# Stalfoes/dqn_mgsc_zoo

Hardware: AMD Instinct MI355X
Metric: learner grad-steps/sec at batch=32, 84×84×4 uint8, 1/2/4/8 MI355X (higher is better)
Workload: dtype f32

## Files before the change

### dqn_mgsc_zoo_amd/_native.py

```python

import ctypes
import glob
import hashlib
import os
import threading

_HERE = os.path.dirname(os.path.abspath(__file__))
LIB_PATH = os.environ.get('DQZ_LIB') or os.path.join(_HERE, 'libdqz.so')
HEADER_PATH = os.path.join(os.path.dirname(_HERE), 'include', 'dqz.h')

DQZ_OK = 0
ALGO_DQN = 0
ALGO_DOUBLE = 1
ALGO_PER = 2
NUM_LEAVES = 10
NUM_PHASES = 10
PHASE_NAMES = (
    'conv1_fwd', 'conv2_fwd', 'conv3_fwd', 'fc1_fwd', 'head', 'fc1_dx',
    'conv3_dx+conv2_dx+fc1_dw+conv3_dw+conv2_dw+conv1_dw', 'unused7',
    'unused8', 'update')
FRAME_H = 84
FRAME_W = 84
STACK = 4
FRAME_BYTES = FRAME_H * FRAME_W
# ... 159 lines not shown
        _int,
        [_vp, ctypes.POINTER(DqzParams), ctypes.POINTER(DqzStore), _vp, _vp,
         ctypes.c_uint64, _vp, _vp, _vp, _vp]),
    'dqz_learner_step_per_draw': (
        _int,
        [_vp, ctypes.POINTER(DqzParams), ctypes.POINTER(DqzStore),
         ctypes.POINTER(DqzPerDraw), _vp]),
    'dqz_learner_grad': (
        _int,
        [_vp, ctypes.POINTER(DqzParams), ctypes.POINTER(DqzStore), _vp, _vp,
         _vp, _vp],
    ),
    'dqz_learner_outputs': (_int, [_vp, _vp, _vp, _vp, _vp]),
    'dqz_learner_sync_status': (_int, [_vp, _vp]),
    'dqz_learner_debug_stall': (_int, [_vp, _int, ctypes.c_uint]),
    'dqz_learner_debug_activations': (_int, [_vp, _int] + [_vp] * 10),
    'dqz_per_write_back': (_int, [_vp, _vp, _i64, _vp, ctypes.c_double, _vp, _vp]),
    'dqz_learner_profile': (
        _int,
        [_vp, ctypes.POINTER(DqzParams), ctypes.POINTER(DqzStore), _vp, _vp,
         _int, ctypes.POINTER(ctypes.c_float), _vp],
    ),
    'dqz_forward': (_int, [_vp, _vp, _vp, _int, _vp, _vp]),
    'dqz_forward_slots': (
        _int, [_vp, _vp, ctypes.POINTER(DqzStore), _vp, _int, _int, _vp, _vp]),
    'dqz_act': (
        _int, [_vp, _vp, _vp, _int, ctypes.c_double, ctypes.c_uint64,
               ctypes.c_uint64, _vp, _vp]),
    'dqz_store_put': (
        _int, [ctypes.POINTER(DqzStore), ctypes.POINTER(DqzTransitionPut), _vp,
# ... 134 lines not shown
```

### dqn_mgsc_zoo_amd/csrc/bwd.hpp

```cpp
#pragma once
#include "common.hpp"
#include "conv1.hpp"
#include "fwd.hpp"
#include "head.hpp"
#include "sampling.hpp"

namespace dqz {

struct Fc1BwdArgs {
  const float* dz1;
  const float* y3;
  float *th, *mu, *nu;
  int64_t w_off;
  Rms rms;
  int B;
  float* dy3;
  const float *w3, *w2;
  float *w3p, *w2p;
};

__device__ __forceinline__ int w3p_src(int i) {
  const int j = i & 3, kq = (i >> 2) & 3, n = (i >> 4) & 15, w = (i >> 8) & 3, r = i >> 10;
  const int tp = r % 9, nq = r / 9;
  return ((8 - tp) * C3CI + 16 * nq + n) * C3CO + 16 * w + 4 * j + kq;
}
__device__ __forceinline__ int w2p_src(int i) {
  const int j = i & 3, kq = (i >> 2) & 3, n = (i >> 4) & 15, w = (i >> 8) & 3, tp = (i >> 10) & 3;
  const int hh = (i >> 12) & 1, pw = (i >> 13) & 1, ph = (i >> 14) & 1;
  const int kh = ph + 2 * (1 - (tp >> 1)), kw = pw + 2 * (1 - (tp & 1));
  return ((kh * C2K + kw) * C2CI + 16 * hh + n) * C2CO + 16 * w + 4 * j + kq;
}
constexpr int W3P_N = 4 * 9 * 1024, W2P_N = 8 * 4 * 1024;

// ... 48 lines not shown
        xacc[mt] = mfma4(av.w, wv[j].w, xacc[mt]);
      }
    }
#pragma unroll
    for (int mt = 0; mt < 2; ++mt)
#pragma unroll
      for (int r = 0; r < 4; ++r) s_red[w][mt][red_at(4 * kq + r, n)] = xacc[mt][r];
    __syncthreads();
#pragma unroll
    for (int h = 0; h < 2; ++h) {
      const int sample = c + 16 * h + (t >> 4);
      const int k = red_at(t >> 4, t & 15);
      const float v2 = (s_red[0][h][k] + s_red[1][h][k]) + (s_red[2][h][k] + s_red[3][h][k]);
      if (sample < a.B) a.dy3[(int64_t)sample * FLAT + k0 + (t & 15)] = ym[h] > 0.f ? v2 : 0.f;
    }
  }
  DQZ_STAMP(5, 3);
}

constexpr int C3X_S = 66, C3X_RS = 754, C3X_WIN = 11 * C3X_RS;
constexpr int C3W_S = 80, C3W_RS = 720, C3W_WIN = 9 * C3W_RS;

struct Conv3BwdArgs {
  const float* dy3;
  const float* y2;
  const float* w3;
  const float* w3p;
  float* dy2;
  float* part;
  int B;
// ... 500 lines not shown
  }
  DQZ_STAMP(11, 3);
}


constexpr int FC1X_BLOCKS = FLAT / 16;
inline int fc1_dx_blocks(int B) { return FC1X_BLOCKS * ((B + 31) / 32); }
__device__ __forceinline__ void fc1_dx_block(const Fc1BwdArgs& a, float* smem, int blk) {
  const int g = blk * 256 + threadIdx.x;
  float v3 = 0.f, v2 = 0.f;
  if (a.w3p) {
    if (g < W3P_N) v3 = a.w3[w3p_src(g)];
    if (g < W2P_N) v2 = a.w2[w2p_src(g)];
  }
  const int kb = blk % FC1X_BLOCKS, c = 32 * (blk / FC1X_BLOCKS);
  fc1_dx_body(a, smem, kb, c, min(c + 32, a.B));
  if (a.w3p) {
    if (g < W3P_N) a.w3p[g] = v3;
    if (g < W2P_N) a.w2p[g] = v2;
  }
  DQZ_STAMP(5, 3);
}

constexpr int FC1X1_ROWS = 32;
constexpr int FC1X1_BLOCKS = FLAT / FC1X1_ROWS;

template <int AMAX, int SMAX, int ZMAX>
__global__ __launch_bounds__(512) void head_dx1_kernel(HeadArgs h, Fc1BwdArgs a) {
  __shared__ __attribute__((aligned(16))) float s_dz[HID];
  DQZ_STAMP(5, 0);
  const int half = threadIdx.x >> 8, t = threadIdx.x & 255;
// ... 22 lines not shown
    d = __fmaf_rn(wv[j].z, z.z, d);
    d = __fmaf_rn(wv[j].w, z.w, d);
  }
  d += dpp_f<0xB1>(d);
  d += dpp_f<0x4E>(d);
  d += dpp_f<0x141>(d);
  d += dpp_f<0x140>(d);
  if ((t & 15) == 0) a.dy3[r] = ym > 0.f ? d : 0.f;
  if (a.w3p) {
    if (g < W3P_N) a.w3p[g] = v3;
    if (g < W2P_N) a.w2p[g] = v2;
  }
  DQZ_STAMP(5, 3);
}

#ifdef DQZ_STEP_TU
inline hipError_t launch_head_dx1(const HeadArgs& h, const Fc1BwdArgs& f, hipStream_t st) {
  if (h.S > 7 || h.Z < 1 || h.Z > 3 || h.B != 1) return hipErrorInvalidValue;
  const dim3 grid(FC1X1_BLOCKS), block(512);
  if (h.A <= 8) {
    if (h.Z <= 2)
      hipLaunchKernelGGL((head_dx1_kernel<8, 7, 2>), grid, block, 0, st, h, f);
    else
      hipLaunchKernelGGL((head_dx1_kernel<8, 7, 3>), grid, block, 0, st, h, f);
  } else {
    if (h.Z <= 2)
      hipLaunchKernelGGL((head_dx1_kernel<MAXA, 7, 2>), grid, block, 0, st, h, f);
    else
      hipLaunchKernelGGL((head_dx1_kernel<MAXA, 7, 3>), grid, block, 0, st, h, f);
  }
  return hipGetLastError();
}
#endif

DQZ_STEP_KERNEL __launch_bounds__(256) void fc1_dx_kernel(Fc1BwdArgs a) {
  __shared__ __attribute__((aligned(16))) float smem[FC1X_SMEM];
  fc1_dx_block(a, smem, blockIdx.x);
}

template <bool WB>
__global__ __launch_bounds__(256) __attribute__((amdgpu_waves_per_eu(4, 8))) void bwd_bc_kernel(
    Conv3BwdArgs c3, Fc1BwdArgs f1, Conv2BwdArgs c2, Conv1DwArgs c1, PerWbArgs wb) {
  constexpr int kW = C3X_WIN > FC1W_SMEM ? C3X_WIN : FC1W_SMEM;
  constexpr int kW2 = C2X_WIN > C3W_WIN ? C2X_WIN : C3W_WIN;
  constexpr int kW3 = C2V_WIN > C1H_SMEM ? C2V_WIN : C1H_SMEM;
  constexpr int kWA = kW > kW2 ? kW : kW2;
  constexpr int kSmem = kWA > kW3 ? kWA : kW3;
  static_assert(kSmem * 4 >= PWB_LDS_BYTES, "the write-back's LDS comes out of the backward's buffer");
  __shared__ __attribute__((aligned(16))) float smem[kSmem];
  const int B8 = (c3.B + 7) / 8 * 8;
// ... 60 lines not shown
```

### dqn_mgsc_zoo_amd/csrc/common.hpp

```cpp
#pragma once
#include <hip/hip_runtime.h>

#include <cstdarg>
#include <cstdint>
#include <cstdio>
#include <string>

#include "dqz.h"

namespace dqz {

typedef float f32x4 __attribute__((ext_vector_type(4)));

#define DQZ_STR(x) #x
#define DQZ_XSTR(x) DQZ_STR(x)
typedef float f32x16 __attribute__((ext_vector_type(16)));

#ifdef DQZ_STEP_TU
#define DQZ_STEP_KERNEL __global__
#define DQZ_OTHER_KERNEL template <int = 0> __global__
#else
#define DQZ_STEP_KERNEL template <int = 0> __global__
#define DQZ_OTHER_KERNEL __global__
#endif
// ... 221 lines not shown
        __builtin_amdgcn_s_sleep(4);
        if (++spins > spin_max) {
          __hip_atomic_fetch_or(err, 1, __ATOMIC_RELAXED, __HIP_MEMORY_SCOPE_AGENT);
          break;
        }
      }
      if (__hip_atomic_fetch_add(ack + b * kStride, 1, __ATOMIC_RELAXED, __HIP_MEMORY_SCOPE_AGENT) == consumers - 1) {
        __hip_atomic_store(cnt + b * kStride, 0, __ATOMIC_RELAXED, __HIP_MEMORY_SCOPE_AGENT);
        __hip_atomic_store(ack + b * kStride, 0, __ATOMIC_RELAXED, __HIP_MEMORY_SCOPE_AGENT);
      }
    }
    __syncthreads();
  }
};

__device__ __forceinline__ float4 load_sc1_f4(const float4* base, int bytes, int e) {
  typedef unsigned u32x4 __attribute__((ext_vector_type(4)));
  const __amdgpu_buffer_rsrc_t r = __builtin_amdgcn_make_buffer_rsrc((void*)base, 0, bytes, 0x00020000);
  return __builtin_bit_cast(float4, __builtin_amdgcn_raw_buffer_load_b128(r, e * 16, 0, 16));
}

__device__ __forceinline__ float load_sc1_f1(const float* base, int bytes, int e) {
  const __amdgpu_buffer_rsrc_t r = __builtin_amdgcn_make_buffer_rsrc((void*)base, 0, bytes, 0x00020000);
  return __builtin_bit_cast(float, __builtin_amdgcn_raw_buffer_load_b32(r, e * 4, 0, 16));
}

__device__ __forceinline__ void store_sc1_f4(float* base, int bytes, int off, f32x4 v) {
  typedef unsigned u32x4 __attribute__((ext_vector_type(4)));
  const __amdgpu_buffer_rsrc_t r = __builtin_amdgcn_make_buffer_rsrc((void*)base, 0, bytes, 0x00020000);
  __builtin_amdgcn_raw_buffer_store_b128(__builtin_bit_cast(u32x4, v), r, off, 0, 16);
// ... 25 lines not shown
```

### dqn_mgsc_zoo_amd/csrc/head.hpp

```cpp
#pragma once
#include "common.hpp"

namespace dqz {

struct HeadArgs {
  const float* fc1p;
  int S;
  float* h1;
  NetZ nz;
  int64_t b1_off, w2_off, b2_off;
  int Z, B, A, algo, shared_bias, fwd_only;
  const int32_t* slots;
  const int32_t* action;
  const float* reward;
  const float* discount;
  const float* weights;
  const double* per_wb;
  int per_normalize;
  float* per_w_out;
  const float* meta_p;
  const float* meta_logits;
  const int32_t* meta_pos;
  int meta_M;
  float *meta_x_out, *meta_p_out;
  const float4* rec;
  uint64_t* advance;
  int unit;
  float bound;
  float* q;
  float* td;
  float* loss_part;
  float* gq;
  int32_t* ga;
  float* dz1;
  dqz_action* act_out;
  double eps;
  uint64_t act_seed, act_ctr;
};

__device__ __forceinline__ dqz_action eps_greedy(const float* q, int A, double eps, double u) {
  float v = q[0];
  for (int a = 1; a < A; ++a) v = fmaxf(v, q[a]);
  int ties = 0;
  for (int a = 0; a < A; ++a) ties += q[a] == v;
  const double greedy = 1.0 / (double)ties, floor = eps / (double)A;
  double total = 0.0;
  for (int a = 0; a < A; ++a) total += (1.0 - eps) * (q[a] == v ? greedy : 0.0) + floor;
  double cum = 0.0;
  int act = A - 1;
// ... 7 lines not shown
  return dqz_action{act, v};
}

__device__ __forceinline__ double wave_max_nonneg(double m) {
  m = fmax(m, dpp_d<0x111>(m));
  m = fmax(m, dpp_d<0x112>(m));
  m = fmax(m, dpp_d<0x114>(m));
  m = fmax(m, dpp_d<0x118>(m));
  m = fmax(m, dpp_d<0x142, 0xa>(m));
  m = fmax(m, dpp_d<0x143, 0xc>(m));
  const long long b = __builtin_bit_cast(long long, m);
  const int lo = __builtin_amdgcn_readlane((int)b, 63), hi = __builtin_amdgcn_readlane((int)(b >> 32), 63);
  return __builtin_bit_cast(double, ((long long)hi << 32) | (unsigned)lo);
}

template <int AMAX, int SMAX, int ZMAX>
__device__ __forceinline__ void head_body(const HeadArgs& h, int b, bool out = true, float* s_dzo = nullptr) {
  DQZ_STAMP(4, 0);
  __shared__ float s_red[8][3 * AMAX];
  __shared__ float s_q[3][AMAX];
  __shared__ float s_rec[5];
  const int n = threadIdx.x, lane = n & 63, wave = n >> 6;
  const int A = h.A, B = h.B, Z = h.Z, S = h.S;
  int a_tm1 = 0;
  float r = 0.f, d = 0.f, w = 1.f, pm = 0.f;
  const bool chain = !h.fwd_only && h.rec == nullptr;
  const int slot = chain ? h.slots[b] : 0;
  float4 rv = make_float4(0.f, 0.f, 0.f, 0.f);
  if (!h.fwd_only && h.rec != nullptr && n == 0) rv = h.rec[b];
  float pv[ZMAX][SMAX], b1v[ZMAX], w2v[ZMAX][AMAX];
#pragma unroll
  for (int z = 0; z < ZMAX; ++z) {
    const int zc = min(z, Z - 1);
    const float* part = h.fc1p + ((int64_t)zc * S * B + b) * HID + n;
#pragma unroll
    for (int s = 0; s < SMAX; ++s) pv[z][s] = part[(int64_t)min(s, S - 1) * B * HID];
    b1v[z] = h.nz.p[zc][h.b1_off + n];
    const float* w2 = h.nz.p[zc] + h.w2_off + n * A;
#pragma unroll
    for (int a = 0; a < AMAX; ++a) w2v[z][a] = w2[min(a, A - 1)];
  }
  constexpr bool kTr = AMAX <= 8;
  constexpr int kPS = HID + 16;
  __shared__ float s_p[kTr ? 3 * AMAX : 1][kTr ? kPS : 1];
  const int K = Z * A, lgT = K <= 16 ? 5 : 4, T = 1 << lgT;
  const int kk = n >> lgT, jj = n & (T - 1);
  const bool qthread = kTr ? (kk < K && jj == 0) : (n < 3 * AMAX && n / AMAX < Z && n % AMAX < A);
  const int zq = kTr ? min(kk / A, 2) : n / AMAX, aq = kTr ? kk % A : n % AMAX;
  float b2v = 0.f;
  {
    const int a2 = h.shared_bias ? 0 : min(aq, A - 1);
    float b2z[ZMAX];
#pragma unroll
    for (int z = 0; z < ZMAX; ++z) b2z[z] = h.nz.p[min(z, Z - 1)][h.b2_off + a2];
    const int zc = min(zq, Z - 1);
#pragma unroll
    for (int z = 0; z < ZMAX; ++z) b2v = zc == z ? b2z[z] : b2v;
  }
  float wper = 1.f;
// ... 67 lines not shown
      if (z == 0) DQZ_STAMP(15, 0);
      if constexpr (kTr) {
#pragma unroll
        for (int a = 0; a < AMAX; ++a)
          if (a < A) s_p[z * A + a][n] = hz[z] * w2v[z][a];
      } else {
#pragma unroll
        for (int a = 0; a < AMAX; ++a) {
          const float sa = wave_sum(hz[z] * w2v[z][a]);
          if (lane == 0) s_red[wave][z * AMAX + a] = sa;
        }
      }
    }
  }
  DQZ_STAMP(15, 1);
  __syncthreads();
  float qv = 0.f;
  if constexpr (kTr) {
    if (kk < K) {
      const float* row = &s_p[kk][jj];
      float a4[4] = {0.f, 0.f, 0.f, 0.f};
      for (int i = 0; i < (HID >> lgT); i += 4) {
#pragma unroll
        for (int u = 0; u < 4; ++u) a4[u] += row[(i + u) << lgT];
      }
      float v = (a4[0] + a4[1]) + (a4[2] + a4[3]);
      v += dpp_f<0xB1>(v);
      v += dpp_f<0x4E>(v);
      v += dpp_f<0x141>(v);
      v += dpp_f<0x140>(v);
// ... 42 lines not shown
          }
        v = q1[0];
#pragma unroll
        for (int a = 1; a < AMAX; ++a) v = a == am ? q1[a] : v;
      }
      const float td = __fmaf_rn(d, v, r) - qa;
      float g;
      if (h.unit) {
        g = -1.f;
      } else if (h.meta_p || h.meta_logits) {
        g = pm * fminf(fmaxf(td, -h.bound), h.bound);
      } else {
        g = w * td / (float)B;
        g = fminf(fmaxf(g, -h.bound), h.bound);
      }
      if (out && n == 0) {
        h.td[b] = td;
        h.loss_part[b] = 0.5f * td * td * w;
        h.gq[b] = -g;
        h.ga[b] = a_tm1;
      }
      float wv = w2v[0][0];
#pragma unroll
      for (int a = 1; a < AMAX; ++a) wv = a == a_tm1 ? w2v[0][a] : wv;
      DQZ_STAMP(4, 2);
      const float dz = hz[0] > 0.f ? -g * wv : 0.f;
      if (s_dzo) s_dzo[n] = dz;
      if (out) h.dz1[(int64_t)b * HID + n] = dz;
    }
  } else if (h.act_out) {
// ... 371 lines not shown
```

### dqn_mgsc_zoo_amd/csrc/learner.hip

```cpp
#include <hip/hip_runtime.h>

#include <algorithm>
#include <array>
#include <functional>
#include <cmath>
#include <vector>
#include <cstdlib>
#include <cstring>

#include "learner_impl.hpp"
#include "meta.hpp"
#include "hvp.hpp"
#include "preprocess.hpp"
#include "census.hpp"

using namespace dqz;

static int g_meta_attr_done = 0;

static int init_meta_attrs() {
  if (g_meta_attr_done) return DQZ_OK;
  DQZ_HIP(hipFuncSetAttribute((const void*)tangent_fwd_kernel, hipFuncAttributeMaxDynamicSharedMemorySize,
                              (int)kConv1FwdSmem));
  g_meta_attr_done = 1;
// ... 1017 lines not shown
  DQZ_HIP(hipGetLastError());
  if (keep) return chunk_sums(logit_buf, logits, true, st);
  return DQZ_OK;
}

int dqz_meta_sync_status(dqz_meta* H, int* status) {
  if (!H || !status) return fail(DQZ_ERR_INVALID, "null argument");
  int s_lm = 0, s_l1 = 0, s_own = 0;
  if (int rc = dqz_learner_sync_status(H->lm, &s_lm)) return rc;
  if (int rc = dqz_learner_sync_status(H->l1, &s_l1)) return rc;
  DQZ_HIP(hipMemcpy(&s_own, H->arrive + 4 * Handoff::kStride, sizeof(int), hipMemcpyDeviceToHost));
  *status = s_lm | s_l1 | s_own;
  if (*status != 0) {
    DQZ_HIP(hipMemset(H->arrive, 0, sizeof(int) * 5 * Handoff::kStride));
    for (dqz_learner* L : {H->lm, H->l1})
      DQZ_HIP(hipMemset(L->sync, 0, sizeof(int) * ((16 * L->cfg.batch + 3) * Handoff::kStride + 64)));
    DQZ_HIP(hipDeviceSynchronize());
  }
  return DQZ_OK;
}

int dqz_meta_debug_stall(dqz_meta* H, int poison, unsigned spin_max) {
  if (!H) return fail(DQZ_ERR_INVALID, "null meta handle");
  const unsigned sm = spin_max ? spin_max : 1u << 24;
  H->spin_max = sm;
  H->lm->spin_max = sm;
  H->l1->spin_max = sm;
  if (poison) {
    const int32_t p = -(1 << 30);
    DQZ_HIP(hipDeviceSynchronize());
    DQZ_HIP(hipMemcpy(H->arrive + Handoff::kStride, &p, sizeof(p), hipMemcpyHostToDevice));
// ... 138 lines not shown
```

### dqn_mgsc_zoo_amd/csrc/learner_impl.hpp

```cpp
#pragma once
#include <hip/hip_runtime.h>

#include <cstring>

#include "common.hpp"
#include "conv1.hpp"
#include "fwd.hpp"
#include "head.hpp"
#include "bwd.hpp"
#include "sampling.hpp"

namespace dqz {

inline void param_layout(int A, int shared_bias, int64_t off[10], int64_t sz[10], int64_t* total) {
  const int64_t sizes[10] = {C1KK * C1CO, C1CO, C2KK * C2CO, C2CO, C3KK * C3CO, C3CO,
                             (int64_t)FLAT * HID, HID, (int64_t)HID * A, shared_bias ? 1 : A};
  int64_t o = 0;
  for (int i = 0; i < 10; ++i) {
    off[i] = o;
    sz[i] = sizes[i];
    o += (sizes[i] + 63) / 64 * 64;
  }
  *total = o;
}

}

struct dqz_learner {
  dqz_learner_config cfg;
  int Z, shared_bias;
  int64_t off[10], sz[10], total;
  int S_fc1, S2, S3;
  float *y1, *y2, *y3, *fc1p, *h1, *q, *dz1, *dy3, *dy2, *dy1, *p1, *p2, *p3, *td, *loss, *loss_part, *gq, *rec;
  float *w3p, *w2p;
  double* per_wb;
  int32_t* ga;
  int32_t* sync;
  unsigned spin_max = 1u << 24;
  void* block;
};


namespace dqz {

inline int check_store(const dqz_store* S) {
  if (!S || !S->frames || !S->fidx || !S->action || !S->reward || !S->discount)
    return fail(DQZ_ERR_INVALID, "store has a null buffer");
  if (S->capacity < 1) return fail(DQZ_ERR_INVALID, "store capacity must be positive");
  return DQZ_OK;
}

inline int device_view(const void* p, const void** out, const char* what) {
  hipPointerAttribute_t attr;
  if (hipPointerGetAttributes(&attr, p) != hipSuccess) {
    (void)hipGetLastError();
    return fail(DQZ_ERR_INVALID, "%s must be device memory or pinned host memory", what);
  }
  if (attr.type == hipMemoryTypeHost) {
// ... 34 lines not shown
```

### dqn_mgsc_zoo_amd/csrc/learner_step.hip

```cpp
#define DQZ_STEP_TU 1
#include <hip/hip_runtime.h>

#include <cstdlib>
#include <cstring>

#include "learner_impl.hpp"

using namespace dqz;

static int g_attr_done = 0;

static int init_kernel_attrs() {
  if (g_attr_done) return DQZ_OK;
  const void* fwd_kernels[] = {(const void*)fwd_conv_kernel<0>, (const void*)fwd_conv_kernel<1>,
                               (const void*)fwd_conv_kernel<2>, (const void*)fwd_conv_kernel<3>,
                               (const void*)fwd_conv_kernel<4>};
  for (const void* k : fwd_kernels)
    DQZ_HIP(hipFuncSetAttribute(k, hipFuncAttributeMaxDynamicSharedMemorySize, (int)kConv1FwdSmem));
  g_attr_done = 1;
  return DQZ_OK;
}

extern "C" {

// ... 15 lines not shown
  L->cfg = *cfg;
  L->Z = cfg->algo == DQZ_ALGO_DQN ? 2 : 3;
  L->shared_bias = cfg->algo == DQZ_ALGO_DQN ? 0 : 1;
  param_layout(cfg->num_actions, L->shared_bias, L->off, L->sz, &L->total);
  const int B = cfg->batch, Z = L->Z, A = cfg->num_actions;
  L->S_fc1 = FC1_S;
  L->S2 = B;
  L->S3 = B;
  const int64_t n_y1 = (int64_t)Z * B * C1M * C1CO, n_y2 = (int64_t)Z * B * C2M * C2CO, n_y3 = (int64_t)Z * B * FLAT;
  const int64_t n_fc1p = (int64_t)Z * L->S_fc1 * B * HID, n_h1 = (int64_t)Z * B * HID, n_q = (int64_t)Z * B * A;
  const int64_t n_dz1 = (int64_t)B * HID, n_dy3 = (int64_t)B * FLAT, n_dy2 = (int64_t)B * C2M * C2CO,
                n_dy1 = (int64_t)B * C1M * C1CO;
  const int64_t n_p1 = (int64_t)B * C1_BLOCKS * (C1KK + 1) * C1CO, n_p2 = (int64_t)L->S2 * (C2KK + 1) * C2CO,
                n_p3 = (int64_t)L->S3 * (C3KK + 1) * C3CO;
  const int64_t sizes[] = {n_y1, n_y2, n_y3, n_fc1p, n_h1, n_q, n_dz1, n_dy3, n_dy2, n_dy1,
                           n_p1, n_p2, n_p3, B,      1,    B,   B,     B,  4 * B, (16 * B + 3) * Handoff::kStride + 64, W3P_N, W2P_N,
                           2 * (int64_t)B};
  float** ptrs[] = {&L->y1,  &L->y2,  &L->y3,  &L->fc1p, &L->h1,   &L->q,         &L->dz1, &L->dy3,
                    &L->dy2, &L->dy1, &L->p1,  &L->p2,   &L->p3,   &L->td,        &L->loss, &L->loss_part,
                    &L->gq,  reinterpret_cast<float**>(&L->ga), &L->rec, reinterpret_cast<float**>(&L->sync), &L->w3p, &L->w2p,
                    reinterpret_cast<float**>(&L->per_wb)};
  static_assert(sizeof(sizes) / sizeof(sizes[0]) == sizeof(ptrs) / sizeof(ptrs[0]), "scratch table");
  int64_t total = 0;
  for (int64_t s : sizes) total += (s + 63) / 64 * 64;
  if (hipMalloc(&L->block, total * sizeof(float)) != hipSuccess) {
    delete L;
    return fail(DQZ_ERR_HIP, "hipMalloc of %lld bytes failed", (long long)(total * 4));
  }
  if (hipMemset(L->block, 0, total * sizeof(float)) != hipSuccess) {
    (void)hipFree(L->block);
    delete L;
    return fail(DQZ_ERR_HIP, "hipMemset of learner scratch failed");
  }
  float* p = (float*)L->block;
  for (size_t i = 0; i < sizeof(sizes) / sizeof(sizes[0]); ++i) {
    *ptrs[i] = p;
// ... 207 lines not shown

  Fc1BwdArgs fb{};
  fb.dz1 = L->dz1;
  fb.y3 = L->y3;
  fb.th = P->online;
  fb.mu = P->mu;
  fb.nu = P->nu;
  fb.w_off = L->off[6];
  fb.rms = rms;
  fb.B = B;
  fb.dy3 = L->dy3;
  fb.w3 = P->online + L->off[4];
  fb.w2 = P->online + L->off[2];
  fb.w3p = L->w3p;
  fb.w2p = L->w2p;
  if (B == 1 && !pe.on()) {
    DQZ_HIP(launch_head_dx1(h, fb, st));
  } else {
    DQZ_PHASE(4, DQZ_HIP(launch_head(h, B, st)));
    DQZ_PHASE(5, hipLaunchKernelGGL(fc1_dx_kernel, dim3(fc1_dx_blocks(B)), dim3(256), 0, st, fb);
              DQZ_HIP(hipGetLastError()));
  }

  Conv3BwdArgs c3b{};
  c3b.dy3 = L->dy3;
  c3b.y2 = L->y2;
  c3b.w3 = P->online + L->off[4];
  c3b.w3p = L->w3p;
  c3b.dy2 = L->dy2;
  c3b.part = L->p3;
  c3b.B = B;
  int* const herr = L->sync + 16 * B * Handoff::kStride;
// ... 106 lines not shown
  for (int i = 0; i < DQZ_NUM_PHASES; ++i) phase_ms[i] = 0.f;
  PhaseEvents pe{nullptr, nullptr, iters, phase_ms};
  DQZ_HIP(hipEventCreate(&pe.e0));
  DQZ_HIP(hipEventCreate(&pe.e1));
  const int rc = step_impl(L, P, S, slots, is_weights, stream, pe);
  (void)hipEventDestroy(pe.e0);
  (void)hipEventDestroy(pe.e1);
  return rc;
}

int dqz_learner_sync_status(dqz_learner* L, int* status) {
  if (!L || !status) return fail(DQZ_ERR_INVALID, "null argument");
  DQZ_HIP(hipDeviceSynchronize());
  DQZ_HIP(hipMemcpy(status, L->sync + 16 * L->cfg.batch * Handoff::kStride, sizeof(int), hipMemcpyDeviceToHost));
  if (*status != 0) {
    DQZ_HIP(hipMemset(L->sync, 0, sizeof(int) * ((16 * L->cfg.batch + 3) * Handoff::kStride + 64)));
    DQZ_HIP(hipDeviceSynchronize());
  }
  return DQZ_OK;
}

int dqz_learner_debug_stall(dqz_learner* L, int sample, unsigned spin_max) {
  if (!L) return fail(DQZ_ERR_INVALID, "null learner");
  if (sample >= L->cfg.batch) return fail(DQZ_ERR_INVALID, "sample out of range");
  L->spin_max = spin_max ? spin_max : 1u << 24;
  if (sample >= 0) {
    const int32_t poison = -(1 << 30);
    DQZ_HIP(hipDeviceSynchronize());
    DQZ_HIP(hipMemcpy(L->sync + (int64_t)sample * Handoff::kStride, &poison, sizeof(poison),
                      hipMemcpyHostToDevice));
  }
  return DQZ_OK;
}

int dqz_learner_outputs(dqz_learner* L, float* q_tm1, float* td, float* loss, void* stream) {
  if (!L) return fail(DQZ_ERR_INVALID, "null learner");
  hipStream_t st = (hipStream_t)stream;
  const int B = L->cfg.batch, A = L->cfg.num_actions;
  if (q_tm1) DQZ_HIP(hipMemcpyAsync(q_tm1, L->q, sizeof(float) * B * A, hipMemcpyDeviceToDevice, st));
  if (td) DQZ_HIP(hipMemcpyAsync(td, L->td, sizeof(float) * B, hipMemcpyDeviceToDevice, st));
  if (loss) DQZ_HIP(hipMemcpyAsync(loss, L->loss, sizeof(float), hipMemcpyDeviceToDevice, st));
  return DQZ_OK;
}

static int forward_q(dqz_learner* L, const float* params, const Conv1Src& src, int which, int n, float* q_out,
                     hipStream_t st) {
// ... 72 lines not shown
```

### dqn_mgsc_zoo_amd/learner.py

```python

import ctypes

import numpy as np
import torch

from dqn_mgsc_zoo_amd import _native
from dqn_mgsc_zoo_amd import networks as networks_lib
from dqn_mgsc_zoo_amd import optim_state

ALGOS = {'dqn': _native.ALGO_DQN, 'double': _native.ALGO_DOUBLE,
         'per': _native.ALGO_PER}


class RMSPropConfig:

  def __init__(self, learning_rate, decay=0.9, eps=1e-8, centered=False):
    if not centered:
      raise NotImplementedError(
          'only centered RMSProp is on the hot path (dqn/run_atari.py:208-213)')
    self.learning_rate = float(learning_rate)
    self.decay = float(decay)
    self.eps = float(eps)
    self.centered = True

# ... 139 lines not shown

  def fetch_outputs(self, stream=None):
    _native.check(_native.lib().dqz_learner_outputs(
        self._h, _native.ptr(self.q_tm1), _native.ptr(self.td),
        _native.ptr(self.loss), _native.stream_handle(stream)))
    return self.q_tm1, self.td, self.loss

  def sync_status(self):
    st = ctypes.c_int(0)
    _native.check(_native.lib().dqz_learner_sync_status(self._h, ctypes.byref(st)))
    return st.value

  def debug_stall(self, sample, spin_max=0):
    _native.check(_native.lib().dqz_learner_debug_stall(self._h, int(sample), int(spin_max)))

  def fetch_activations(self, z=0, backward=False, stream=None):
    b, a = self.batch_size, self.network.num_actions
    shapes = dict(y1=(b, 20, 20, 32), y2=(b, 9, 9, 64), y3=(b, 7, 7, 64),
                  h1=(b, 512), q=(b, a))
    if backward:
      shapes.update(dz1=(b, 512), dy3=(b, 7, 7, 64), dy2=(b, 9, 9, 64),
                    dy1=(b, 20, 20, 32))
    out = {k: torch.empty(s, dtype=torch.float32, device=self.device)
           for k, s in shapes.items()}
    _native.check(_native.lib().dqz_learner_debug_activations(
        self._h, int(z),
        *(_native.ptr(out.get(k)) for k in ('y1', 'y2', 'y3', 'h1', 'q', 'dz1',
                                             'dy3', 'dy2', 'dy1')),
        _native.stream_handle(stream)))
    return out
# ... 188 lines not shown
```

### include/dqz.h

```cpp
#ifndef DQZ_H_
#define DQZ_H_

#include <stdint.h>

#ifdef __cplusplus
extern "C" {
#endif

#define DQZ_OK 0
#define DQZ_ERR_INVALID (-1)
#define DQZ_ERR_HIP (-2)
#define DQZ_ERR_UNSUPPORTED (-3)

#define DQZ_ALGO_DQN 0
#define DQZ_ALGO_DOUBLE 1
#define DQZ_ALGO_PER 2

#define DQZ_FRAME_H 84
#define DQZ_FRAME_W 84
#define DQZ_STACK 4
#define DQZ_FRAME_BYTES (DQZ_FRAME_H * DQZ_FRAME_W)
#define DQZ_NUM_LEAVES 10

const char* dqz_last_error(void);
// ... 58 lines not shown

int dqz_learner_grad(dqz_learner* learner, const dqz_params* params, const dqz_store* store,
                     const int32_t* slots, const float* is_weights, float* grad_out, void* stream);

#define DQZ_NUM_PHASES 10

int dqz_learner_profile(dqz_learner* learner, const dqz_params* params, const dqz_store* store,
                        const int32_t* slots, const float* is_weights, int iters, float* phase_ms,
                        void* stream);

int dqz_learner_outputs(dqz_learner* learner, float* q_tm1, float* td, float* loss, void* stream);

int dqz_learner_sync_status(dqz_learner* learner, int* status);

int dqz_learner_debug_stall(dqz_learner* learner, int sample, unsigned spin_max);

int dqz_learner_debug_activations(dqz_learner* learner, int z, float* y1, float* y2, float* y3, float* h1,
                                  float* q, float* dz1, float* dy3, float* dy2, float* dy1, void* stream);

int dqz_forward(dqz_learner* learner, const float* params, const uint8_t* states, int n,
                float* q_out, void* stream);

int dqz_forward_slots(dqz_learner* learner, const float* params, const dqz_store* store,
                      const int32_t* slots, int n, int which, float* q_out, void* stream);

typedef struct dqz_action {
  int32_t action;
  float value;
} dqz_action;
int dqz_act(dqz_learner* learner, const float* params, const uint8_t* states, int n, double epsilon,
// ... 159 lines not shown
```

Baseline: 16300.

## Merge head and fc1 dx into one kernel with compact dz record handoff

Adds a merged head_dx kernel. The first B workgroups run the head and publish a compact per-sample record (negated grad, action, ReLU mask bits) through an atomic counter handoff. The remaining workgroups rebuild dz1 on the fly from W2 rows and the mask, then compute fc1 dx, so one kernel launch and the dense dz1 round trip are removed. It risks spin-wait deadlock and deliberately pads LDS so only one workgroup fits per CU, which lowers occupancy.

```diff
diff --git a/dqn_mgsc_zoo_amd/_native.py b/dqn_mgsc_zoo_amd/_native.py
--- a/dqn_mgsc_zoo_amd/_native.py
+++ b/dqn_mgsc_zoo_amd/_native.py
@@ -197,6 +197,7 @@
     'dqz_learner_outputs': (_int, [_vp, _vp, _vp, _vp, _vp]),
     'dqz_learner_sync_status': (_int, [_vp, _vp]),
     'dqz_learner_debug_stall': (_int, [_vp, _int, ctypes.c_uint]),
+    'dqz_learner_debug_head_path': (_int, [_vp, _int]),
     'dqz_learner_debug_activations': (_int, [_vp, _int] + [_vp] * 10),
     'dqz_per_write_back': (_int, [_vp, _vp, _i64, _vp, ctypes.c_double, _vp, _vp]),
     'dqz_learner_profile': (
diff --git a/dqn_mgsc_zoo_amd/csrc/bwd.hpp b/dqn_mgsc_zoo_amd/csrc/bwd.hpp
--- a/dqn_mgsc_zoo_amd/csrc/bwd.hpp
+++ b/dqn_mgsc_zoo_amd/csrc/bwd.hpp
@@ -17,6 +17,9 @@
   float* dy3;
   const float *w3, *w2;
   float *w3p, *w2p;
+  const float* hrec;
+  const float* w2h;
+  int A;
 };
 
 __device__ __forceinline__ int w3p_src(int i) {
@@ -95,6 +98,164 @@
       const float v2 = (s_red[0][h][k] + s_red[1][h][k]) + (s_red[2][h][k] + s_red[3][h][k]);
       if (sample < a.B) a.dy3[(int64_t)sample * FLAT + k0 + (t & 15)] = ym[h] > 0.f ? v2 : 0.f;
     }
+  }
+  DQZ_STAMP(5, 3);
+}
+
+constexpr int FC1X_RA = 8;
+constexpr int FC1X_W2LD = HID + 8;
+constexpr int FC1X_W2T = FC1X_RA * FC1X_W2LD;
+constexpr int FC1X_REC_SMEM = FC1X_W2T + 4 * 2 * FC1X_RED + HID * FC1X_RA;
+
+constexpr int FC1X_W2NAT = HID * FC1X_RA;
+template <int NT>
+struct Fc1W2Regs {
+  static constexpr int N = (HID * FC1X_RA / 4 + NT - 1) / NT;
+  float4 v[N];
+  __device__ __forceinline__ void load(const Fc1BwdArgs& a, int t) {
+#pragma unroll
+    for (int k = 0; k < N; ++k) v[k] = reinterpret_cast<const float4*>(a.w2h)[min(t + NT * k, 128 * a.A - 1)];
+  }
+  __device__ __forceinline__ void store(const Fc1BwdArgs& a, float* s_nat, int t) const {
+#pragma unroll
+    for (int k = 0; k < N; ++k) reinterpret_cast<float4*>(s_nat)[min(t + NT * k, 128 * a.A - 1)] = v[k];
+  }
+  static __device__ __forceinline__ void to_tile(const Fc1BwdArgs& a, const float* s_nat, float* s_w2t, int t) {
+    float x[HID / NT][FC1X_RA];
+#pragma unroll
+    for (int k = 0; k < HID / NT; ++k)
+#pragma unroll
+      for (int aa = 0; aa < FC1X_RA; ++aa) x[k][aa] = s_nat[(t + NT * k) * a.A + min(aa, a.A - 1)];
+#pragma unroll
+    for (int k = 0; k < HID / NT; ++k)
+#pragma unroll
+      for (int aa = 0; aa < FC1X_RA; ++aa) s_w2t[aa * FC1X_W2LD + t + NT * k] = x[k][aa];
+  }
+};
+
+template <bool SC1>
+__device__ __forceinline__ float4 fc1_rec_ld(const Fc1BwdArgs& a, int q) {
+  if constexpr (SC1)
+    return load_sc1_f4(reinterpret_cast<const float4*>(a.hrec), a.B * 128, q);
+  else
+    return reinterpret_cast<const float4*>(a.hrec)[q];
+}
+
+__device__ __forceinline__ void fc1_rec_keep(float4& v) {
+  asm volatile("" : "+v"(v.x), "+v"(v.y), "+v"(v.z), "+v"(v.w));
+}
+
+template <int NM>
+struct Fc1RecRegs {
+  float gq[NM];
+  int ai[NM];
+  unsigned mw[NM][4];
+  template <bool SC1>
+  __device__ __forceinline__ void load(const Fc1BwdArgs& a, int c, int mt0, int n, int kq, int w) {
+    float4 g[NM], m[NM][2];
+#pragma unroll
+    for (int mt = 0; mt < NM; ++mt) {
+      const int q = 8 * min(c + 16 * (mt0 + mt) + n, a.B - 1);
+      g[mt] = fc1_rec_ld<SC1>(a, q);
+      m[mt][0] = fc1_rec_ld<SC1>(a, q + w);
+      m[mt][1] = fc1_rec_ld<SC1>(a, q + w + 1);
+    }
+    if constexpr (SC1) {
+#pragma unroll
+      for (int mt = 0; mt < NM; ++mt) {
+        fc1_rec_keep(g[mt]);
+        fc1_rec_keep(m[mt][0]);
+        fc1_rec_keep(m[mt][1]);
+      }
+    }
+#pragma unroll
+    for (int mt = 0; mt < NM; ++mt) {
+      const bool in = c + 16 * (mt0 + mt) + n < a.B;
+      const int ar = __float_as_int(g[mt].y);
+      gq[mt] = g[mt].x;
+      ai[mt] = ar < 1 || ar >= FC1X_RA ? 0 : ar;
+      const float mf[4] = {m[mt][0].z, m[mt][0].w, m[mt][1].x, m[mt][1].y};
+#pragma unroll
+      for (int i = 0; i < 4; ++i) mw[mt][i] = in ? __float_as_uint(mf[i]) >> (4 * kq) : 0u;
+    }
+  }
+};
+
+__device__ __forceinline__ float fc1_rec_dz(float gq, float w, unsigned word, int bit) {
+  const unsigned keep = (unsigned)((int)(word << (31 - bit)) >> 31);
+  return __uint_as_float(__float_as_uint(gq * w) & keep);
+}
+
+template <int NM>
+__device__ __forceinline__ void fc1_dx_rec_tail(const Fc1BwdArgs& a, const float* s_w2t,
+                                                float (*s_red)[2][FC1X_RED], int k0, int c, int mt0, int t,
+                                                const float4 (&wv)[8], const float (&ym)[NM],
+                                                const Fc1RecRegs<NM>& r) {
+  auto red_at = [](int row, int col) { return row * 16 + 16 * (row >> 2) + col; };
+  const int lane = t & 63, w = t >> 6;
+  const int n = lane & 15, kq = lane >> 4;
+  f32x4 xacc[NM];
+#pragma unroll
+  for (int mt = 0; mt < NM; ++mt) xacc[mt] = f32x4{0.f, 0.f, 0.f, 0.f};
+#pragma unroll
+  for (int mt = 0; mt < NM; ++mt) {
+    const float* d = s_w2t + r.ai[mt] * FC1X_W2LD + 128 * w + 4 * kq;
+    const float gq = r.gq[mt];
+#pragma unroll
+    for (int j = 0; j < 8; ++j) {
+      const float4 wq = *reinterpret_cast<const float4*>(d + 16 * j);
+      const unsigned word = r.mw[mt][j >> 1];
+      const int b0 = 16 * (j & 1);
+      xacc[mt] = mfma4(fc1_rec_dz(gq, wq.x, word, b0), wv[j].x, xacc[mt]);
+      xacc[mt] = mfma4(fc1_rec_dz(gq, wq.y, word, b0 + 1), wv[j].y, xacc[mt]);
+      xacc[mt] = mfma4(fc1_rec_dz(gq, wq.z, word, b0 + 2), wv[j].z, xacc[mt]);
+      xacc[mt] = mfma4(fc1_rec_dz(gq, wq.w, word, b0 + 3), wv[j].w, xacc[mt]);
+    }
+  }
+#pragma unroll
+  for (int mt = 0; mt < NM; ++mt)
+#pragma unroll
+    for (int rr = 0; rr < 4; ++rr) s_red[w][mt0 + mt][red_at(4 * kq + rr, n)] = xacc[mt][rr];
+  __syncthreads();
+#pragma unroll
+  for (int i = 0; i < NM; ++i) {
+    const int h = mt0 + i;
+    const int sample = c + 16 * h + (t >> 4);
+    const int k = red_at(t >> 4, t & 15);
+    const float v2 = (s_red[0][h][k] + s_red[1][h][k]) + (s_red[2][h][k] + s_red[3][h][k]);
+    if (sample < a.B) a.dy3[(int64_t)sample * FLAT + k0 + (t & 15)] = ym[i] > 0.f ? v2 : 0.f;
+  }
+}
+
+__device__ __forceinline__ void fc1_dx_rec_body(const Fc1BwdArgs& a, float* smem, int blk, int c_beg, int c_end) {
+  DQZ_STAMP(5, 0);
+  float* s_w2t = smem;
+  float(*s_red)[2][FC1X_RED] = reinterpret_cast<float(*)[2][FC1X_RED]>(smem + FC1X_W2T);
+  float* s_nat = smem + FC1X_W2T + 4 * 2 * FC1X_RED;
+  const int t = threadIdx.x, lane = t & 63, w = t >> 6;
+  const int n = lane & 15, kq = lane >> 4;
+  const int k0 = 16 * blk;
+  const float* W1 = a.th + a.w_off;
+  float4 wv[8];
+#pragma unroll
+  for (int j = 0; j < 8; ++j)
+    wv[j] = *reinterpret_cast<const float4*>(W1 + (int64_t)(k0 + n) * HID + 128 * w + 16 * j + 4 * kq);
+  Fc1W2Regs<256> w2r;
+  w2r.load(a, t);
+  for (int c = c_beg; c < c_end; c += 32) {
+    Fc1RecRegs<2> r;
+    r.load<false>(a, c, 0, n, kq, w);
+    float ym[2];
+#pragma unroll
+    for (int h = 0; h < 2; ++h)
+      ym[h] = a.y3[(int64_t)min(c + 16 * h + (t >> 4), a.B - 1) * FLAT + k0 + (t & 15)];
+    if (c == c_beg) {
+      w2r.store(a, s_nat, t);
+      __syncthreads();
+      Fc1W2Regs<256>::to_tile(a, s_nat, s_w2t, t);
+    }
+    __syncthreads();
+    fc1_dx_rec_tail<2>(a, s_w2t, s_red, k0, c, 0, t, wv, ym, r);
   }
   DQZ_STAMP(5, 3);
 }
@@ -625,7 +786,10 @@
     if (g < W2P_N) v2 = a.w2[w2p_src(g)];
   }
   const int kb = blk % FC1X_BLOCKS, c = 32 * (blk / FC1X_BLOCKS);
-  fc1_dx_body(a, smem, kb, c, min(c + 32, a.B));
+  if (a.hrec)
+    fc1_dx_rec_body(a, smem, kb, c, min(c + 32, a.B));
+  else
+    fc1_dx_body(a, smem, kb, c, min(c + 32, a.B));
   if (a.w3p) {
     if (g < W3P_N) a.w3p[g] = v3;
     if (g < W2P_N) a.w2p[g] = v2;
@@ -678,7 +842,73 @@
   DQZ_STAMP(5, 3);
 }
 
+constexpr int HDX_BLOCKS = FLAT / 16;
+constexpr int HDX_DX = FC1X_W2T + 4 * 2 * FC1X_RED;
+constexpr int HDX_NEED = HDX_DX > 3 * 8 * HEAD_PS ? HDX_DX : 3 * 8 * HEAD_PS;
+constexpr int CU_LDS_FLOATS = 160 * 1024 / 4;
+constexpr int HDX_PAD = CU_LDS_FLOATS / 2 + 512;
+constexpr int HDX_SMEM = HDX_NEED > HDX_PAD ? HDX_NEED : HDX_PAD;
+static_assert(2 * HDX_SMEM > CU_LDS_FLOATS && HDX_SMEM <= CU_LDS_FLOATS, "exactly one head_dx_kernel workgroup fits a CU");
+static_assert(FC1X_W2T + FC1X_W2NAT <= HDX_SMEM, "W2 as loaded sits behind the tile");
+
+template <int SMAX, int ZMAX>
+__global__ __launch_bounds__(512) void head_dx_kernel(HeadArgs h, Fc1BwdArgs a, HandoffR hand) {
+  __shared__ __attribute__((aligned(16))) float smem[HDX_SMEM];
+  if ((int)blockIdx.x < h.B) {
+    head_body<8, SMAX, ZMAX, true>(h, blockIdx.x, true, nullptr, &hand, smem);
+    return;
+  }
+  DQZ_STAMP(5, 0);
+  const int blk = blockIdx.x - h.B;
+  const int half = threadIdx.x >> 8, t = threadIdx.x & 255;
+  const int lane = t & 63, w = t >> 6;
+  const int n = lane & 15, kq = lane >> 4;
+  const int k0 = 16 * blk;
+  float* s_w2t = smem;
+  float(*s_red)[2][FC1X_RED] = reinterpret_cast<float(*)[2][FC1X_RED]>(smem + FC1X_W2T);
+  float* s_nat = smem + FC1X_W2T;
+  const float* W1 = a.th + a.w_off;
+  float4 wv[8];
+#pragma unroll
+  for (int j = 0; j < 8; ++j)
+    wv[j] = *reinterpret_cast<const float4*>(W1 + (int64_t)(k0 + n) * HID + 128 * w + 16 * j + 4 * kq);
+  Fc1W2Regs<512> w2r;
+  w2r.load(a, threadIdx.x);
+  float ym[1];
+  ym[0] = a.y3[(int64_t)min(16 * half + (t >> 4), a.B - 1) * FLAT + k0 + (t & 15)];
+  const int g = blk * 256 + t;
+  float v3 = 0.f, v2 = 0.f;
+  if (a.w3p && half == 0) {
+    if (g < W3P_N) v3 = a.w3[w3p_src(g)];
+    if (g < W2P_N) v2 = a.w2[w2p_src(g)];
+  }
+  w2r.store(a, s_nat, threadIdx.x);
+  if (a.w3p && half == 0) {
+    if (g < W3P_N) a.w3p[g] = v3;
+    if (g < W2P_N) a.w2p[g] = v2;
+  }
+  __syncthreads();
+  Fc1W2Regs<512>::to_tile(a, s_nat, s_w2t, threadIdx.x);
+  hand.wait(blk);
+  DQZ_STAMP(5, 1);
+  Fc1RecRegs<1> r;
+  r.load<true>(a, 0, half, n, kq, w);
+  fc1_dx_rec_tail<1>(a, s_w2t, s_red, k0, 0, half, t, wv, ym, r);
+  DQZ_STAMP(5, 3);
+}
+
 #ifdef DQZ_STEP_TU
+inline hipError_t launch_head_dx(const HeadArgs& h, const Fc1BwdArgs& f, const HandoffR& hand, hipStream_t st) {
+  if (h.S > 7 || h.Z < 1 || h.Z > 3 || h.B < 2 || h.B > 32 || h.A > FC1X_RA || !h.hrec || !f.hrec)
+    return hipErrorInvalidValue;
+  const dim3 grid(h.B + HDX_BLOCKS), block(512);
+  if (h.Z <= 2)
+    hipLaunchKernelGGL((head_dx_kernel<7, 2>), grid, block, 0, st, h, f, hand);
+  else
+    hipLaunchKernelGGL((head_dx_kernel<7, 3>), grid, block, 0, st, h, f, hand);
+  return hipGetLastError();
+}
+
 inline hipError_t launch_head_dx1(const HeadArgs& h, const Fc1BwdArgs& f, hipStream_t st) {
   if (h.S > 7 || h.Z < 1 || h.Z > 3 || h.B != 1) return hipErrorInvalidValue;
   const dim3 grid(FC1X1_BLOCKS), block(512);
@@ -698,6 +928,7 @@
 #endif
 
 DQZ_STEP_KERNEL __launch_bounds__(256) void fc1_dx_kernel(Fc1BwdArgs a) {
+  static_assert(FC1X_REC_SMEM <= FC1X_SMEM, "the record path's LDS comes out of the dz1 chunk's");
   __shared__ __attribute__((aligned(16))) float smem[FC1X_SMEM];
   fc1_dx_block(a, smem, blockIdx.x);
 }
diff --git a/dqn_mgsc_zoo_amd/csrc/common.hpp b/dqn_mgsc_zoo_amd/csrc/common.hpp
--- a/dqn_mgsc_zoo_amd/csrc/common.hpp
+++ b/dqn_mgsc_zoo_amd/csrc/common.hpp
@@ -259,6 +259,41 @@
   }
 };
 
+struct HandoffR {
+  static constexpr int R = 32;
+  int* cnt;
+  int* ack;
+  int* err;
+  int need, consumers;
+  unsigned spin_max = 1u << 24;
+  __device__ __forceinline__ void arrive(int) const {
+    asm volatile("s_waitcnt vmcnt(0)" ::: "memory");
+    __syncthreads();
+    if (threadIdx.x < R)
+      __hip_atomic_fetch_add(cnt + threadIdx.x * Handoff::kStride, 1, __ATOMIC_RELAXED, __HIP_MEMORY_SCOPE_AGENT);
+  }
+  __device__ __forceinline__ void wait(int j) const {
+    if (threadIdx.x == 0) {
+      const int rep = j % R, mine = (consumers - rep + R - 1) / R;
+      int* c = cnt + rep * Handoff::kStride;
+      int* k = ack + rep * Handoff::kStride;
+      unsigned spins = 0;
+      while (__hip_atomic_load(c, __ATOMIC_RELAXED, __HIP_MEMORY_SCOPE_AGENT) < need) {
+        __builtin_amdgcn_s_sleep(4);
+        if (++spins > spin_max) {
+          __hip_atomic_fetch_or(err, 1, __ATOMIC_RELAXED, __HIP_MEMORY_SCOPE_AGENT);
+          break;
+        }
+      }
+      if (__hip_atomic_fetch_add(k, 1, __ATOMIC_RELAXED, __HIP_MEMORY_SCOPE_AGENT) == mine - 1) {
+        __hip_atomic_store(c, 0, __ATOMIC_RELAXED, __HIP_MEMORY_SCOPE_AGENT);
+        __hip_atomic_store(k, 0, __ATOMIC_RELAXED, __HIP_MEMORY_SCOPE_AGENT);
+      }
+    }
+    __syncthreads();
+  }
+};
+
 __device__ __forceinline__ float4 load_sc1_f4(const float4* base, int bytes, int e) {
   typedef unsigned u32x4 __attribute__((ext_vector_type(4)));
   const __amdgpu_buffer_rsrc_t r = __builtin_amdgcn_make_buffer_rsrc((void*)base, 0, bytes, 0x00020000);
diff --git a/dqn_mgsc_zoo_amd/csrc/head.hpp b/dqn_mgsc_zoo_amd/csrc/head.hpp
--- a/dqn_mgsc_zoo_amd/csrc/head.hpp
+++ b/dqn_mgsc_zoo_amd/csrc/head.hpp
@@ -33,6 +33,7 @@
   float* gq;
   int32_t* ga;
   float* dz1;
+  float* hrec;
   dqz_action* act_out;
   double eps;
   uint64_t act_seed, act_ctr;
@@ -70,8 +71,10 @@
   return __builtin_bit_cast(double, ((long long)hi << 32) | (unsigned)lo);
 }
 
-template <int AMAX, int SMAX, int ZMAX>
-__device__ __forceinline__ void head_body(const HeadArgs& h, int b, bool out = true, float* s_dzo = nullptr) {
+constexpr int HEAD_PS = HID + 16;
+template <int AMAX, int SMAX, int ZMAX, bool EXT = false>
+__device__ __forceinline__ void head_body(const HeadArgs& h, int b, bool out = true, float* s_dzo = nullptr,
+                                          const HandoffR* pub = nullptr, float* s_ext = nullptr) {
   DQZ_STAMP(4, 0);
   __shared__ float s_red[8][3 * AMAX];
   __shared__ float s_q[3][AMAX];
@@ -97,8 +100,10 @@
     for (int a = 0; a < AMAX; ++a) w2v[z][a] = w2[min(a, A - 1)];
   }
   constexpr bool kTr = AMAX <= 8;
-  constexpr int kPS = HID + 16;
-  __shared__ float s_p[kTr ? 3 * AMAX : 1][kTr ? kPS : 1];
+  constexpr int kPS = HEAD_PS;
+  __shared__ float s_p_own[kTr && !EXT ? 3 * AMAX : 1][kTr ? kPS : 1];
+  float(*s_p)[kTr ? kPS : 1] = EXT ? reinterpret_cast<float(*)[kTr ? kPS : 1]>(s_ext) : s_p_own;
+  __shared__ unsigned s_hm[16];
   const int K = Z * A, lgT = K <= 16 ? 5 : 4, T = 1 << lgT;
   const int kk = n >> lgT, jj = n & (T - 1);
   const bool qthread = kTr ? (kk < K && jj == 0) : (n < 3 * AMAX && n / AMAX < Z && n % AMAX < A);
@@ -196,6 +201,13 @@
     }
   }
   DQZ_STAMP(15, 1);
+  if (h.hrec) {
+    const unsigned long long m = __ballot(hz[0] > 0.f);
+    if (lane == 0) {
+      s_hm[2 * wave] = (unsigned)m;
+      s_hm[2 * wave + 1] = (unsigned)(m >> 32);
+    }
+  }
   __syncthreads();
   float qv = 0.f;
   if constexpr (kTr) {
@@ -268,6 +280,21 @@
         g = w * td / (float)B;
         g = fminf(fmaxf(g, -h.bound), h.bound);
       }
+      if (out && h.hrec && n < 8) {
+        typedef unsigned u32x4 __attribute__((ext_vector_type(4)));
+        u32x4 rv4;
+#pragma unroll
+        for (int e = 0; e < 4; ++e) {
+          const int dw = 4 * n + e - 2;
+          rv4[e] = dw >= 0 && dw < 16 ? s_hm[min(max(dw, 0), 15)] : 0u;
+        }
+        if (n == 0) {
+          rv4[0] = __float_as_uint(-g);
+          rv4[1] = (unsigned)a_tm1;
+        }
+        store_sc1_f4(h.hrec, B * 128, (32 * b + 4 * n) * 4, __builtin_bit_cast(f32x4, rv4));
+      }
+      if (pub) pub->arrive(0);
       if (out && n == 0) {
         h.td[b] = td;
         h.loss_part[b] = 0.5f * td * td * w;
diff --git a/dqn_mgsc_zoo_amd/csrc/learner.hip b/dqn_mgsc_zoo_amd/csrc/learner.hip
--- a/dqn_mgsc_zoo_amd/csrc/learner.hip
+++ b/dqn_mgsc_zoo_amd/csrc/learner.hip
@@ -1055,7 +1055,7 @@
   if (*status != 0) {
     DQZ_HIP(hipMemset(H->arrive, 0, sizeof(int) * 5 * Handoff::kStride));
     for (dqz_learner* L : {H->lm, H->l1})
-      DQZ_HIP(hipMemset(L->sync, 0, sizeof(int) * ((16 * L->cfg.batch + 3) * Handoff::kStride + 64)));
+      DQZ_HIP(hipMemset(L->sync, 0, sizeof(int) * sync_ints(L->cfg.batch)));
     DQZ_HIP(hipDeviceSynchronize());
   }
   return DQZ_OK;
diff --git a/dqn_mgsc_zoo_amd/csrc/learner_impl.hpp b/dqn_mgsc_zoo_amd/csrc/learner_impl.hpp
--- a/dqn_mgsc_zoo_amd/csrc/learner_impl.hpp
+++ b/dqn_mgsc_zoo_amd/csrc/learner_impl.hpp
@@ -34,14 +34,18 @@
   float *y1, *y2, *y3, *fc1p, *h1, *q, *dz1, *dy3, *dy2, *dy1, *p1, *p2, *p3, *td, *loss, *loss_part, *gq, *rec;
   float *w3p, *w2p;
   double* per_wb;
+  float* hrec;
   int32_t* ga;
   int32_t* sync;
   unsigned spin_max = 1u << 24;
+  int head_path = 2;
   void* block;
 };
 
 
 namespace dqz {
+
+inline int64_t sync_ints(int B) { return (int64_t)(16 * B + 3 + 2 * HandoffR::R) * Handoff::kStride + 64; }
 
 inline int check_store(const dqz_store* S) {
   if (!S || !S->frames || !S->fidx || !S->action || !S->reward || !S->discount)
diff --git a/dqn_mgsc_zoo_amd/csrc/learner_step.hip b/dqn_mgsc_zoo_amd/csrc/learner_step.hip
--- a/dqn_mgsc_zoo_amd/csrc/learner_step.hip
+++ b/dqn_mgsc_zoo_amd/csrc/learner_step.hip
@@ -53,12 +53,12 @@
   const int64_t n_p1 = (int64_t)B * C1_BLOCKS * (C1KK + 1) * C1CO, n_p2 = (int64_t)L->S2 * (C2KK + 1) * C2CO,
                 n_p3 = (int64_t)L->S3 * (C3KK + 1) * C3CO;
   const int64_t sizes[] = {n_y1, n_y2, n_y3, n_fc1p, n_h1, n_q, n_dz1, n_dy3, n_dy2, n_dy1,
-                           n_p1, n_p2, n_p3, B,      1,    B,   B,     B,  4 * B, (16 * B + 3) * Handoff::kStride + 64, W3P_N, W2P_N,
-                           2 * (int64_t)B};
+                           n_p1, n_p2, n_p3, B,      1,    B,   B,     B,  4 * B, sync_ints(B), W3P_N, W2P_N,
+                           2 * (int64_t)B, 32 * (int64_t)B};
   float** ptrs[] = {&L->y1,  &L->y2,  &L->y3,  &L->fc1p, &L->h1,   &L->q,         &L->dz1, &L->dy3,
                     &L->dy2, &L->dy1, &L->p1,  &L->p2,   &L->p3,   &L->td,        &L->loss, &L->loss_part,
                     &L->gq,  reinterpret_cast<float**>(&L->ga), &L->rec, reinterpret_cast<float**>(&L->sync), &L->w3p, &L->w2p,
-                    reinterpret_cast<float**>(&L->per_wb)};
+                    reinterpret_cast<float**>(&L->per_wb), &L->hrec};
   static_assert(sizeof(sizes) / sizeof(sizes[0]) == sizeof(ptrs) / sizeof(ptrs[0]), "scratch table");
   int64_t total = 0;
   for (int64_t s : sizes) total += (s + 63) / 64 * 64;
@@ -296,8 +296,21 @@
   fb.w2 = P->online + L->off[2];
   fb.w3p = L->w3p;
   fb.w2p = L->w2p;
+  const bool merged = L->head_path == 2 && A <= FC1X_RA && B >= 2 && B <= 32 && !pe.on();
+  const bool rec = (merged || L->head_path == 1) && A <= FC1X_RA && !(B == 1 && !pe.on());
+  if (rec) {
+    h.hrec = L->hrec;
+    fb.hrec = L->hrec;
+    fb.w2h = P->online + L->off[8];
+    fb.A = A;
+  }
   if (B == 1 && !pe.on()) {
     DQZ_HIP(launch_head_dx1(h, fb, st));
+  } else if (merged) {
+    int* const hw = L->sync + (16 * B + 3) * Handoff::kStride;
+    const HandoffR hand{hw, hw + HandoffR::R * Handoff::kStride, L->sync + 16 * B * Handoff::kStride, B,
+                        HDX_BLOCKS, L->spin_max};
+    DQZ_HIP(launch_head_dx(h, fb, hand, st));
   } else {
     DQZ_PHASE(4, DQZ_HIP(launch_head(h, B, st)));
     DQZ_PHASE(5, hipLaunchKernelGGL(fc1_dx_kernel, dim3(fc1_dx_blocks(B)), dim3(256), 0, st, fb);
@@ -434,7 +447,7 @@
   DQZ_HIP(hipDeviceSynchronize());
   DQZ_HIP(hipMemcpy(status, L->sync + 16 * L->cfg.batch * Handoff::kStride, sizeof(int), hipMemcpyDeviceToHost));
   if (*status != 0) {
-    DQZ_HIP(hipMemset(L->sync, 0, sizeof(int) * ((16 * L->cfg.batch + 3) * Handoff::kStride + 64)));
+    DQZ_HIP(hipMemset(L->sync, 0, sizeof(int) * sync_ints(L->cfg.batch)));
     DQZ_HIP(hipDeviceSynchronize());
   }
   return DQZ_OK;
@@ -450,6 +463,13 @@
     DQZ_HIP(hipMemcpy(L->sync + (int64_t)sample * Handoff::kStride, &poison, sizeof(poison),
                       hipMemcpyHostToDevice));
   }
+  return DQZ_OK;
+}
+
+int dqz_learner_debug_head_path(dqz_learner* L, int mode) {
+  if (!L) return fail(DQZ_ERR_INVALID, "null learner");
+  if (mode < 0 || mode > 2) return fail(DQZ_ERR_INVALID, "head path mode must be 0, 1 or 2");
+  L->head_path = mode;
   return DQZ_OK;
 }
 
diff --git a/dqn_mgsc_zoo_amd/learner.py b/dqn_mgsc_zoo_amd/learner.py
--- a/dqn_mgsc_zoo_amd/learner.py
+++ b/dqn_mgsc_zoo_amd/learner.py
@@ -177,6 +177,9 @@
   def debug_stall(self, sample, spin_max=0):
     _native.check(_native.lib().dqz_learner_debug_stall(self._h, int(sample), int(spin_max)))
 
+  def debug_head_path(self, mode):
+    _native.check(_native.lib().dqz_learner_debug_head_path(self._h, int(mode)))
+
   def fetch_activations(self, z=0, backward=False, stream=None):
     b, a = self.batch_size, self.network.num_actions
     shapes = dict(y1=(b, 20, 20, 32), y2=(b, 9, 9, 64), y3=(b, 7, 7, 64),
diff --git a/include/dqz.h b/include/dqz.h
--- a/include/dqz.h
+++ b/include/dqz.h
@@ -96,6 +96,8 @@
 int dqz_learner_sync_status(dqz_learner* learner, int* status);
 
 int dqz_learner_debug_stall(dqz_learner* learner, int sample, unsigned spin_max);
+
+int dqz_learner_debug_head_path(dqz_learner* learner, int mode);
 
 int dqz_learner_debug_activations(dqz_learner* learner, int z, float* y1, float* y2, float* y3, float* h1,
                                   float* q, float* dz1, float* dy3, float* dy2, float* dy1, void* stream);
```

Result: no change. 16310 (median of 2 runs) (+0.1%).
